# cristicbz/rust-doom

Hardware: NVIDIA H100
Metric: frames/sec at 1920x1080 (palette-index bit-exact) (higher is better)
Workload: dtype u8

## Files before the change

### rust-doom_b200/csrc/b2d_kernels.cu

```cuda
#include "b2d_kernels.cuh"

namespace b2d {

namespace {

constexpr unsigned kFull = 0xFFFFFFFFu;

constexpr int kMaskWords = 128;
constexpr int kStackDepth = 128;

constexpr uint32_t kVisBit = 1u << 25, kSolidBit = 1u << 24;
__device__ __forceinline__ uint32_t pack_range(int lo, int hi, uint32_t bits) {
    return (uint32_t)lo | ((uint32_t)hi << 12) | bits;
}
__device__ __forceinline__ int range_lo(uint32_t r) { return (int)(r & 0xFFFu); }
__device__ __forceinline__ int range_hi(uint32_t r) { return (int)((r >> 12) & 0xFFFu); }

__device__ __forceinline__ uint32_t word_bits(int w, int lo, int hi) {
    int a = max(lo, w * 32), b = min(hi, w * 32 + 31);
    if (a > b) return 0u;
    uint32_t m = 0xFFFFFFFFu >> (31 - (b - w * 32));
    return m & (0xFFFFFFFFu << (a - w * 32));
}

// ... 413 lines not shown
        const uint32_t r = sc.skyrow[y];
        put_px<kRgba>(c, p8, p32, y >= ya && y < yb, __ldg(px + (inter ? (r >> 2) * w4 + (r & 3u) : r * T.w)));
    }
}

template <bool kRgba, int kW>
__device__ __forceinline__ void draw_plane_warp(const RasterCtx &c, const FrameConst &fc, const View &vw,
                                                int ya, int yb, int32_t h, int32_t flat, int lightb,
                                                bool visible) {
    const DeviceScene &sc = *c.sc;
    if (!__any_sync(kFull, ya < yb)) return;
    if (!visible) { fill_void_warp<kRgba, kW>(c, ya, yb); return; }
    if (flat == kFlatSky) { draw_sky_warp<kRgba, kW>(c, ya, yb); return; }
    if (flat < 0 || flat >= sc.nflats) { fill_void_warp<kRgba, kW>(c, ya, yb); return; }
    const uint64_t px_hi = reinterpret_cast<uint64_t>(sc.lit_flats) & 0xFFFFFFFF00000000ull;
    const uint32_t habs = plane_habs(h, fc.pose.z);
    bool act = ya < yb;
    int y0 = __reduce_min_sync(kFull, act ? ya : 0x7FFFFFFF);
    int y1 = __reduce_max_sync(kFull, act ? yb : 0);
    const int full_lo = __reduce_max_sync(kFull, act ? ya : 0x7FFFFFFF);
    const int full_hi = __reduce_min_sync(kFull, act ? yb : 0);
    const int Wc = kW ? kW : c.W;
    uint8_t *p8 = c.fb + (size_t)y0 * Wc;
    uint32_t *p32 = kRgba ? c.rgba + (size_t)y0 * Wc : nullptr;
    const uint32_t bu = (uint32_t)fc.pose.x << 10, bv = (uint32_t)fc.pose.y << 10;
    const uint32_t ax = (uint32_t)c.dir.ax, ay = (uint32_t)c.dir.ay;
    for (int yc = y0; yc < y1; yc += 32) {
        int yy = yc + c.lane;
        if (yy < y1) {
            const PlaneRow pr = plane_row(habs, sc.yslope[yy]);
            c.rowz[c.lane] = make_uint2(pr.z8q, (sc.lit_flat_stride >> 6) * (uint32_t)light_row(lightb, pr.z8) + 64u * (uint32_t)flat);
        }
        __syncwarp();
        const int rows = min(32, y1 - yc);
        int j = 0;
        for (; j + kBatch <= rows; j += kBatch, p8 += (size_t)kBatch * Wc, p32 += (size_t)kBatch * Wc) {
            uint32_t v[kBatch];
#pragma unroll
            for (int k = 0; k < kBatch; k++) {
                const uint2 rz = c.rowz[j + k];
                v[k] = __ldg(reinterpret_cast<const uint8_t *>(px_hi | flat_offset(rz.y, bu + rz.x * ax, bv + rz.x * ay)));
            }
            const int y = yc + j;
            store_batch<kRgba, kW>(c, p8, p32, v, y, ya, yb, y >= full_lo && y + kBatch <= full_hi);
        }
        for (; j < rows; j++, p8 += Wc, p32 += Wc) {
            const uint2 rz = c.rowz[j];
            const int y = yc + j;
            put_px<kRgba>(c, p8, p32, y >= ya && y < yb,
                          __ldg(reinterpret_cast<const uint8_t *>(px_hi | flat_offset(rz.y, bu + rz.x * ax, bv + rz.x * ay))));
        }
        __syncwarp();
    }
}

template <bool kRgba, int kW, int R>
__device__ __forceinline__ void wall_fast_loop(const RasterCtx &c, const uint8_t *plq, uint32_t w4, uint32_t nq, uint32_t q,
                                               uint32_t acc, uint32_t ts29, int y0, int y1, int ya, int yb,
                                               int full_lo, int full_hi) {
    const int Wc = kW ? kW : c.W;
    uint8_t *p8 = c.fb + (size_t)y0 * Wc;
    uint32_t *p32 = kRgba ? c.rgba + (size_t)y0 * Wc : nullptr;
    asm("" : "+l"(plq));
#pragma unroll 1
    for (int y = y0; y < y1; y += R, p8 += (size_t)R * Wc, p32 += (size_t)R * Wc) {
        const uint32_t q1 = q + 1u == nq ? 0u : q + 1u;
        const uint32_t w0 = __ldg(reinterpret_cast<const uint32_t *>(plq + (size_t)q * w4));
        const uint32_t w1 = __ldg(reinterpret_cast<const uint32_t *>(plq + (size_t)q1 * w4));
        if (y >= full_lo && y + R <= full_hi) {
#pragma unroll
            for (int k = 0; k < R; k++) {
                uint32_t v = pick_byte(w0, w1, wall_sel(acc, ts29, (uint32_t)k));
                if (kRgba) v &= 0xFFu;
                put_px<kRgba>(c, p8 + (size_t)k * Wc, kRgba ? p32 + (size_t)k * Wc : nullptr, true, v);
            }
        } else {
            const uint32_t m = row_mask(y, ya, yb, R);
#pragma unroll
            for (int k = 0; k < R; k++) {
                uint32_t v = pick_byte(w0, w1, wall_sel(acc, ts29, (uint32_t)k));
                if (kRgba) v &= 0xFFu;
                put_px<kRgba>(c, p8 + (size_t)k * Wc, kRgba ? p32 + (size_t)k * Wc : nullptr, (m >> k) & 1u, v);
            }
        }
        wall_advance(acc, q, ts29, (uint32_t)R, nq);
    }
}

template <bool kRgba, int kW>
__device__ __forceinline__ void draw_wall_warp(const RasterCtx &c, const FrameConst &fc, int ya, int yb,
                                               int32_t tex, int32_t tA, int32_t hA, int32_t ucol,
                                               int32_t iscale, int row) {
    const DeviceScene &sc = *c.sc;
    if (!__any_sync(kFull, ya < yb)) return;
    if (tex < 0 || tex >= sc.ntex) { fill_void_warp<kRgba, kW>(c, ya, yb); return; }
    const TexRec T = sc.tex[tex];
    bool act = ya < yb;
    const uint32_t col = (uint32_t)floormod32(ucol, (int32_t)T.w);
    const uint8_t *pl = sc.lit_texels + (size_t)row * sc.lit_texel_stride + T.texel_off;
    const uint32_t tstep = (uint32_t)(iscale >> 4);
    int y0 = __reduce_min_sync(kFull, act ? ya : 0x7FFFFFFF);
    int y1 = __reduce_max_sync(kFull, act ? yb : 0);
    const int full_lo = __reduce_max_sync(kFull, act ? ya : 0x7FFFFFFF);
    const int full_hi = __reduce_min_sync(kFull, act ? yb : 0);
    uint32_t t = (uint32_t)wall_tbase(tA, hA, fc.pose.z, c.H, iscale) + (uint32_t)y0 * tstep;
    const int Wc = kW ? kW : c.W;
    uint8_t *p8 = c.fb + (size_t)y0 * Wc;
    uint32_t *p32 = kRgba ? c.rgba + (size_t)y0 * Wc : nullptr;
    if (tex_interleaved(T) && T.h >= 8u) {
        const uint32_t ts = act ? tstep : 0u;
        const bool f16 = __all_sync(kFull, ts <= kWallFast16);
        if (f16 || __all_sync(kFull, ts <= kWallFast8)) {
            const uint32_t tt = act ? t : 0u;
            const uint32_t r0 = wall_row((int32_t)tt, T.h, T.hmagic, T.hbias);
            const uint8_t *plq = pl + 4u * col;
            if (f16) wall_fast_loop<kRgba, kW, 16>(c, plq, 4u * T.w, T.h >> 2, r0 >> 2, wall_acc29(tt, r0), ts << 13, y0, y1, ya, yb, full_lo, full_hi);
            else wall_fast_loop<kRgba, kW, 8>(c, plq, 4u * T.w, T.h >> 2, r0 >> 2, wall_acc29(tt, r0), ts << 13, y0, y1, ya, yb, full_lo, full_hi);
            return;
        }
    }
    if (tex_interleaved(T)) {
        const uint32_t colb = 4u * col, w4 = 4u * T.w;
        for (int y = y0; y < y1; y += kBatch, p8 += (size_t)kBatch * Wc, p32 += (size_t)kBatch * Wc, t += (uint32_t)kBatch * tstep) {
            const uint32_t r0 = wall_row((int32_t)t, T.h, T.hmagic, T.hbias);
            const uint32_t acc = wall_acc(t, r0);
            const uint32_t b7 = (acc + 7u * tstep) >> 16;
            uint32_t v[kBatch];
            if (__all_sync(kFull, b7 < 8u)) {
                const uint32_t q0 = r0 >> 2, q1 = next_quad(q0, T.h);
                const uint32_t w0 = __ldg(reinterpret_cast<const uint32_t *>(pl + (q0 * w4 + colb)));
                const uint32_t w1 = __ldg(reinterpret_cast<const uint32_t *>(pl + (q1 * w4 + colb)));
#pragma unroll
                for (int k = 0; k < kBatch; k++) {
                    v[k] = pick_byte(w0, w1, (acc + (uint32_t)k * tstep) >> 16);
                    if (kRgba) v[k] &= 0xFFu;
                }
            } else {
                const uint32_t t4 = t + 4u * tstep;
                const uint32_t r4 = wall_row((int32_t)t4, T.h, T.hmagic, T.hbias);
                const uint32_t acc4 = wall_acc(t4, r4);
                if (__all_sync(kFull, ((acc + 3u * tstep) >> 16) < 8u && ((acc4 + 3u * tstep) >> 16) < 8u)) {
                    const uint32_t q0 = r0 >> 2, q4 = r4 >> 2;
                    const uint32_t a0 = __ldg(reinterpret_cast<const uint32_t *>(pl + (q0 * w4 + colb)));
                    const uint32_t a1 = __ldg(reinterpret_cast<const uint32_t *>(pl + (next_quad(q0, T.h) * w4 + colb)));
                    const uint32_t b0 = __ldg(reinterpret_cast<const uint32_t *>(pl + (q4 * w4 + colb)));
                    const uint32_t b1 = __ldg(reinterpret_cast<const uint32_t *>(pl + (next_quad(q4, T.h) * w4 + colb)));
#pragma unroll
                    for (int k = 0; k < 4; k++) {
                        v[k] = pick_byte(a0, a1, (acc + (uint32_t)k * tstep) >> 16);
                        v[k + 4] = pick_byte(b0, b1, (acc4 + (uint32_t)k * tstep) >> 16);
                        if (kRgba) { v[k] &= 0xFFu; v[k + 4] &= 0xFFu; }
                    }
                } else {
#pragma unroll
                    for (int k = 0; k < kBatch; k++) {
                        const uint32_t rk = wall_row((int32_t)(t + (uint32_t)k * tstep), T.h, T.hmagic, T.hbias);
                        v[k] = __ldg(pl + ((rk >> 2) * w4 + colb + (rk & 3u)));
                    }
                }
            }
            store_batch<kRgba, kW>(c, p8, p32, v, y, ya, yb, y >= full_lo && y + kBatch <= full_hi);
        }
    } else {
        const uint8_t *px = pl + col;
#pragma unroll 1
        for (int y = y0; y < y1; y++, p8 += Wc, p32 += Wc, t += tstep)
            put_px<kRgba>(c, p8, p32, y >= ya && y < yb, __ldg(px + wall_row((int32_t)t, T.h, T.hmagic, T.hbias) * T.w));
    }
}

__device__ __forceinline__ uint32_t *masked_entry(const DeviceScene &sc, const uint32_t *chunks, int e) {
    return sc.masked_list + ((size_t)chunks[e / kMaskedChunk] * kMaskedChunk + (size_t)(e % kMaskedChunk)) * 33u;
}
__device__ __forceinline__ uint32_t *masked_push(const DeviceScene &sc, uint32_t *chunks, int &mcount, int lane) {
    bool ok = mcount < sc.masked_cap;
    if (ok && mcount % kMaskedChunk == 0) {
        uint32_t id = 0;
        if (lane == 0) id = atomicAdd(sc.masked_counter, 1u);
        id = __shfl_sync(kFull, id, 0);
        ok = id < sc.masked_chunks;
        if (ok && lane == 0) chunks[mcount / kMaskedChunk] = id;
        __syncwarp();
    }
    if (!ok) {
        if (lane == 0) atomicOr(sc.status_flag, kStatusMaskedFull);
        return nullptr;
    }
    return masked_entry(sc, chunks, mcount++);
}

template <bool kRgba, int kW, bool kStates, bool kLevels>
__device__ __noinline__ void masked_pass(const DeviceScene &sc, const View &vw, int32_t pose_z, uint8_t *fb,
                                         uint32_t *rgba, uint32_t pal_s, int x, int lane,
                                         const SegFrame *wl, const uint32_t *chunks, int count) {
    RasterCtx c;
    c.sc = &sc; c.pal_s = pal_s; c.fb = fb; c.rgba = rgba;
    c.W = vw.W; c.H = vw.H; c.x = x; c.lane = lane;
    const int Wc = kW ? kW : c.W;
    for (int e = count - 1; e >= 0; e--) {
        const uint32_t *ml = masked_entry(sc, chunks, e);
        const uint32_t k = ml[0];
        const uint32_t packed = ml[1 + c.lane];
        int ya = (int)(packed & 0xFFFFu), yb = (int)(packed >> 16);
        const SegFrame sf = wl[k];
        int32_t tex, tA, hA, ucol = 0, iscale = 1, row = 0;
        if (is_sprite_entry(sf)) {
            SpriteFrame sp;
            const SpriteRec P = sc.sprites[entry_sprite(sf, sp)];
            if (P.tex < 0 || P.tex >= sc.ntex) continue;
            const int32_t sw = (int32_t)sc.tex[P.tex].w, sh = (int32_t)sc.tex[P.tex].h;
            const int64_t scale = sprite_scale(vw, sp.cz);
            int32_t z8;
            scale_depth(vw, scale, iscale, z8);
            row = light_row_sprite(P.light, z8);
            tex = P.tex; tA = 0; hA = P.low + sh;
            if (ya < yb) {
                clip_rows(P.low + sh, P.low, row_scale(scale), pose_z, c.H, ya, yb);
                ucol = sprite_column(sp, vw, c.x, sw);
            }
        } else {
            const SegRec S = sc.segs[sf.seg];
            if (S.mid < 0 || S.mid >= sc.nmids) continue;
            const MidRec M = sc.mids[S.mid];
            tex = M.tex; tA = M.t_high; hA = M.high;
            ColumnEval ce = {0u, 1, 1, 0};
            if (ya < yb && column_eval(sf, vw, c.x, ce)) {
                clip_rows(M.high, M.low, ce.scale, pose_z, c.H, ya, yb);
                ucol = wall_column(S.uoff, S.len_q12, ce.s24);
                iscale = ce.iscale;
                row = light_row(S.light, ce.z8);
            } else {
                ya = yb = 0;
            }
        }
        if (tex < 0 || tex >= sc.ntex) continue;
        const TexRec T = sc.tex[tex];
        const bool act = ya < yb;
        int y0 = __reduce_min_sync(kFull, act ? ya : 0x7FFFFFFF);
        int y1 = __reduce_max_sync(kFull, act ? yb : 0);
        if (y0 >= y1) continue;
        const uint32_t col = (uint32_t)floormod32(ucol, (int32_t)T.w);
        const bool inter = tex_interleaved(T);
        const bool has_mask = T.mask_off != 0xFFFFFFFFu;
        const uint8_t *pl = sc.lit_texels + (size_t)row * sc.lit_texel_stride + T.texel_off;
        const uint8_t *pm = sc.lit_texels + (size_t)32 * sc.lit_texel_stride + T.texel_off;
        const uint32_t tstep = (uint32_t)(iscale >> 4);
        uint32_t t = (uint32_t)wall_tbase(tA, hA, pose_z, c.H, iscale) + (uint32_t)y0 * tstep;
        uint8_t *p8 = c.fb + (size_t)y0 * Wc;
        uint32_t *p32 = kRgba ? c.rgba + (size_t)y0 * Wc : nullptr;
        const uint32_t len = act ? (uint32_t)(yb - ya) : 0u;
        if (inter) {
            const uint32_t colb = 4u * col, w4 = 4u * T.w;
#pragma unroll 1
            for (int y = y0; y < y1; y += kBatch, p8 += (size_t)kBatch * Wc, p32 += (size_t)kBatch * Wc, t += (uint32_t)kBatch * tstep) {
                const uint32_t r0 = wall_row((int32_t)t, T.h, T.hmagic, T.hbias);
                const uint32_t acc = wall_acc(t, r0);
                const uint32_t d = (uint32_t)(y - ya);
                uint32_t v[kBatch], o[kBatch];
                if (__all_sync(kFull, ((acc + 7u * tstep) >> 16) < 8u)) {
                    const uint32_t o0 = (r0 >> 2) * w4 + colb, o1 = next_quad(r0 >> 2, T.h) * w4 + colb;
                    const uint32_t w0 = __ldg(reinterpret_cast<const uint32_t *>(pl + o0));
                    const uint32_t w1 = __ldg(reinterpret_cast<const uint32_t *>(pl + o1));
                    uint32_t m0 = 0x01010101u, m1 = 0x01010101u;
                    if (has_mask) {
                        m0 = __ldg(reinterpret_cast<const uint32_t *>(pm + o0));
                        m1 = __ldg(reinterpret_cast<const uint32_t *>(pm + o1));
                    }
#pragma unroll
                    for (int k = 0; k < kBatch; k++) {
                        const uint32_t bk = (acc + (uint32_t)k * tstep) >> 16;
                        v[k] = pick_byte(w0, w1, bk) & 0xFFu;
                        o[k] = pick_byte(m0, m1, bk) & 0xFFu;
                    }
                } else {
#pragma unroll
                    for (int k = 0; k < kBatch; k++) {
                        const uint32_t rk = wall_row((int32_t)(t + (uint32_t)k * tstep), T.h, T.hmagic, T.hbias);
                        const uint32_t off = (rk >> 2) * w4 + colb + (rk & 3u);
                        v[k] = __ldg(pl + off);
                        o[k] = has_mask ? (uint32_t)__ldg(pm + off) : 1u;
                    }
                }
#pragma unroll
                for (int k = 0; k < kBatch; k++)
                    put_px<kRgba>(c, p8 + (size_t)k * Wc, kRgba ? p32 + (size_t)k * Wc : nullptr, d + (uint32_t)k < len && o[k] != 0u, v[k]);
            }
        } else {
#pragma unroll 1
            for (int y = y0; y < y1; y++, p8 += Wc, p32 += Wc, t += tstep) {
                const uint32_t off = wall_row((int32_t)t, T.h, T.hmagic, T.hbias) * T.w + col;
                const bool on = (uint32_t)(y - ya) < len && (!has_mask || __ldg(pm + off) != 0);
                put_px<kRgba>(c, p8, p32, on, __ldg(pl + off));
            }
        }
    }
}

constexpr int kRasterWarps = 8;

constexpr uint32_t kQueueWords = 6144;
constexpr uint32_t kQueueRecs = kQueueWords / 32;
constexpr uint32_t kRecWall = 1u << 16, kRecVisible = 1u << 17;

struct DrawQueue {
    uint4 *head;
    uint32_t *pool;
    uint32_t *nrec, *nwords;
};

__device__ __forceinline__ bool queue_push(const DrawQueue &q, int lane, uint32_t meta, int32_t a, int32_t b, int32_t c,
                                           int ya, int yb, int32_t ucol, uint32_t iscale_row) {
    const bool act = ya < yb;
    if (!__any_sync(kFull, act)) return true;
    const bool wall = meta & kRecWall;
    const uint32_t words = wall ? 96u : 32u;
    uint32_t off = 0, i = kQueueRecs;
    if (lane == 0) {
        off = atomicAdd(q.nwords, words);
        if (off + words <= kQueueWords) i = atomicAdd(q.nrec, 1u);
    }
    i = __shfl_sync(kFull, i, 0);
    if (i >= kQueueRecs) return false;
    off = __shfl_sync(kFull, off, 0);
    q.pool[off + lane] = act ? (uint32_t)ya | ((uint32_t)yb << 16) : 0u;
    if (wall) {
        q.pool[off + 32 + lane] = (uint32_t)ucol;
        q.pool[off + 64 + lane] = iscale_row;
    }
    if (lane == 0) q.head[i] = make_uint4(meta | off, (uint32_t)a, (uint32_t)b, (uint32_t)c);
    return true;
}

template <bool kRgba, int kW, bool kMasked, bool kStates, bool kLevels>
__global__ void __launch_bounds__(32 * kRasterWarps, 16 / kRasterWarps)
b2d_raster_kernel(const __grid_constant__ DeviceScene sc, const __grid_constant__ View vw, const FrameConst *__restrict__ frames,
                  const SegFrame *__restrict__ work, int stride, int n, int strips,
                  uint8_t *__restrict__ index_fb, uint32_t *__restrict__ rgba_fb, const __grid_constant__ StateTables st,
                  const __grid_constant__ LevelTables lt) {
    __shared__ uint32_t s_pal[kRgba ? (kLevels ? 256 * kRasterWarps : 256) : 1];
    __shared__ uint2 s_rowz[kRasterWarps][32];
    __shared__ uint32_t s_chunks[kRasterWarps][kMasked ? kMaskedCapMax / kMaskedChunk : 1];
    __shared__ int4 s_lanes[kRasterWarps][32];
    __shared__ int s_frame[kRasterWarps];
    __shared__ uint4 s_qhead[kQueueRecs];
    __shared__ uint32_t s_qpool[kQueueWords];
    __shared__ uint32_t s_qn[3];
    __shared__ DeviceScene s_scn[kStates || kLevels ? kRasterWarps : 1];
    if (threadIdx.x < 3) s_qn[threadIdx.x] = 0;
    if (kRgba && !kLevels) {
        for (int i = threadIdx.x; i < 256; i += blockDim.x) s_pal[i] = sc.palette[i];
    }
    __syncthreads();

    const int lane = threadIdx.x & 31, warp = threadIdx.x >> 5;
    const long long gw = (long long)blockIdx.x * (blockDim.x >> 5) + warp;
    const bool has_strip = gw < (long long)n * strips;
    const int frame = has_strip ? (int)(gw / strips) : 0, strip = has_strip ? (int)(gw % strips) : 0;
    const int W = kW ? kW : vw.W, H = vw.H;
    const int x0 = strip * 32, x = x0 + lane;
    const bool inside = has_strip && x < W;
    const DrawQueue q{s_qhead, s_qpool, &s_qn[0], &s_qn[1]};

    FrameConst fc{};
    if (has_strip) fc = frames[frame];
    const DeviceScene *scp = &sc;
    if constexpr (kStates && !kLevels) {
        DeviceScene *d = &s_scn[warp];
        if (has_strip) {
            const uint32_t *src = reinterpret_cast<const uint32_t *>(&sc);
            uint32_t *dst = reinterpret_cast<uint32_t *>(d);
            for (int i = lane; i < (int)(sizeof(DeviceScene) / 4); i += 32) dst[i] = src[i];
            __syncwarp();
            if (lane == 0) {
                const uint8_t *tb = st.base + (size_t)(uint32_t)fc.pad[0] * st.slot_bytes;
                d->tex = reinterpret_cast<const TexRec *>(tb);
                d->sectors = reinterpret_cast<const SectorRec *>(tb + st.off_sectors);
                d->segs = reinterpret_cast<const SegRec *>(tb + st.off_segs);
                d->sprites = reinterpret_cast<const SpriteRec *>(tb + st.off_sprites);
                d->mids = reinterpret_cast<const MidRec *>(tb + st.off_mids);
            }
            __syncwarp();
        }
        scp = d;
    }
    if constexpr (kLevels) {
        DeviceScene *d = &s_scn[warp];
        if (has_strip) {
            const DeviceScene *lsrc = lt.scenes + (uint32_t)fc.pad[1];
            const uint32_t *src = reinterpret_cast<const uint32_t *>(lsrc);
            uint32_t *dst = reinterpret_cast<uint32_t *>(d);
            for (int i = lane; i < (int)(sizeof(DeviceScene) / 4); i += 32) dst[i] = src[i];
            if (kRgba) {
                const uint32_t *pal = lsrc->palette;
                for (int i = lane; i < 256; i += 32) s_pal[256 * warp + i] = pal[i];
            }
            __syncwarp();
            if constexpr (kStates) {
                if (lane == 0) {
                    const TableSet t = lt.sets[(uint32_t)fc.pad[0]];
                    d->tex = t.tex; d->sectors = t.sectors; d->segs = t.segs; d->sprites = t.sprites; d->mids = t.mids;
                }
                __syncwarp();
            }
        }
        scp = d;
    }
    const DeviceScene &ts = *scp;
    const DeviceScene &ls = kLevels ? ts : sc;
    RasterCtx c;
    c.sc = &ts;
    c.pal_s = (uint32_t)__cvta_generic_to_shared(kLevels ? s_pal + 256 * warp : s_pal);
    c.rowz = s_rowz[warp];
    c.W = W; c.H = H; c.x = x; c.lane = lane;
    int mcount = 0;
    uint32_t *chunks = s_chunks[warp];
    asm("" : "+l"(chunks));
    const SegFrame *wl = work + (size_t)frame * stride;

    if (has_strip) {
    c.dir = plane_dir(fc, vw, inside ? x : 0, ls.invF);
    c.fb = index_fb + (size_t)frame * W * H + (inside ? x : 0);
    c.rgba = kRgba ? rgba_fb + (size_t)frame * W * H + (inside ? x : 0) : nullptr;
    c.skycol = 0;
    if (ls.sky_tex >= 0 && inside) c.skycol = umulhi32(sky_u32(x, vw, fc.pose.angle), ts.tex[ls.sky_tex].w);
    s_lanes[warp][lane] = make_int4(c.dir.ax, c.dir.ay, (int)c.skycol, inside ? x : 0);
    if (lane == 0) s_frame[warp] = frame;

    int ct = 0, cb = inside ? H : 0;
    const bool defer = kMasked && ls.masked_list != nullptr;
    const int count = fc.count;
    const uint32_t owner = (uint32_t)warp << 18;
    bool done = false;

    for (int k0 = 0; k0 < count && !done; k0 += 32) {
        int k = k0 + lane;
        bool overlap = false;
        if (k < count) {
            int xlo = wl[k].xlo, xhi = wl[k].xhi;
            overlap = xhi >= x0 && xlo <= x0 + 31;
        }
        unsigned m = __ballot_sync(kFull, overlap);
        while (m) {
            int j = __ffs(m) - 1;
            m &= m - 1;
            if (!__any_sync(kFull, ct < cb)) { done = true; break; }
            const SegFrame sf = wl[k0 + j];
            bool in = inside && ct < cb && x >= sf.xlo && x <= sf.xhi;
            if (!__any_sync(kFull, in)) continue;
            if (is_sprite_entry(sf)) {
                if (defer) {
                    uint32_t *ml = masked_push(ls, chunks, mcount, lane);
                    if (ml) {
                        if (lane == 0) ml[0] = (uint32_t)(k0 + j);
                        ml[1 + lane] = in ? ((uint32_t)ct | ((uint32_t)cb << 16)) : 0u;
                    }
                }
                continue;
            }
            ColumnEval ce = {0u, 1, 1, 0};
            bool ok = in && column_eval(sf, vw, x, ce);
            if (!__any_sync(kFull, ok)) continue;

            const SegRec S = ts.segs[sf.seg];
            const SectorRec SF = ts.sectors[S.front];
            const int32_t fcl = SF.ceil, ffl = SF.floor;
            const bool two = S.flags & kSegTwoSided;
            const bool ceil_vis = plane_visible(true, fcl, SF.ceil_flat == kFlatSky, fc.pose.z);
            const bool floor_vis = plane_visible(false, ffl, SF.floor_flat == kFlatSky, fc.pose.z);

            WallRows wr = {ct, ct, ct, ct};
            int yend = ct, row = 0;
            int32_t ucol = 0;
            if (ok) {
                row = light_row(S.light, ce.z8);
                ucol = wall_column(S.uoff, S.len_q12, ce.s24);
                wr = wall_rows(fcl, ffl, two, S.otop, S.obot, ce.scale, fc.pose.z, H, ct, cb);
                yend = cb;
            }
#pragma unroll 1
            for (int pz = 0; pz < 2; pz++) {
                const bool top = pz == 0;
                const int ya = ok ? (top ? ct : wr.y4) : 0, yb = ok ? (top ? wr.y1 : yend) : 0;
                const int32_t h = top ? fcl : ffl, flat = top ? SF.ceil_flat : SF.floor_flat;
                const bool vis = top ? ceil_vis : floor_vis;
                if (!queue_push(q, lane, owner | (vis ? kRecVisible : 0u), h, flat, SF.light, ya, yb, 0, 0u))
                    draw_plane_warp<kRgba, kW>(c, fc, vw, ya, yb, h, flat, SF.light, vis);
            }
#pragma unroll 1
            for (int pw = 0; pw < 2; pw++) {
                const bool upper = pw == 0;
                if (!wall_piece(upper, two, fcl, ffl, S.otop, S.obot)) continue;
                const int ya = ok ? (upper ? wr.y1 : wr.y3) : 0, yb = ok ? (upper ? wr.y2 : wr.y4) : 0;
                const int32_t tex = upper ? S.texA : S.texB, tA = upper ? S.tA : S.tB, hA = upper ? S.hA : S.hB;
                if (!queue_push(q, lane, owner | kRecWall, tex, tA, hA, ya, yb, ucol, (uint32_t)ce.iscale | ((uint32_t)row << 24)))
                    draw_wall_warp<kRgba, kW>(c, fc, ya, yb, tex, tA, hA, ucol, ce.iscale, row);
            }
            if (ok) wall_window(two, wr, H, ct, cb);
            if (defer && two && S.mid >= 0) {
                const bool keep = ok && wr.y2 < wr.y3;
                if (__any_sync(kFull, keep)) {
                    uint32_t *ml = masked_push(ls, chunks, mcount, lane);
                    if (ml) {
                        if (lane == 0) ml[0] = (uint32_t)(k0 + j);
                        ml[1 + lane] = keep ? ((uint32_t)wr.y2 | ((uint32_t)wr.y3 << 16)) : 0u;
                    }
                }
            }
        }
    }
    if (!queue_push(q, lane, owner, 0, 0, 0, inside ? ct : 0, inside ? cb : 0, 0, 0u))
        fill_void_warp<kRgba, kW>(c, inside ? ct : 0, inside ? cb : 0);
    }

    __syncthreads();
    const uint32_t nrec = min(s_qn[0], kQueueRecs);
    for (;;) {
        uint32_t i = 0;
        if (lane == 0) i = atomicAdd(&s_qn[2], 1u);
        i = __shfl_sync(kFull, i, 0);
        if (i >= nrec) break;
        const uint4 hd = s_qhead[i];
        const uint32_t off = hd.x & 0xFFFFu, o = hd.x >> 18;
        const int4 ln = s_lanes[o][lane];
        const int f = s_frame[o];
        const FrameConst fo = frames[f];
        RasterCtx d;
        d.sc = kStates || kLevels ? &s_scn[o] : &sc;
        d.pal_s = (uint32_t)__cvta_generic_to_shared(kLevels ? s_pal + 256 * o : s_pal);
        d.rowz = s_rowz[warp];
        d.dir = PlaneDir{ln.x, ln.y};
        d.fb = index_fb + (size_t)f * W * H + ln.w;
        d.rgba = kRgba ? rgba_fb + (size_t)f * W * H + ln.w : nullptr;
        d.W = W; d.H = H; d.x = ln.w; d.lane = lane;
        d.skycol = (uint32_t)ln.z;
        const uint32_t win = s_qpool[off + lane];
        const int ya = (int)(win & 0xFFFFu), yb = (int)(win >> 16);
        if (hd.x & kRecWall) {
            const uint32_t isr = s_qpool[off + 64 + lane];
            draw_wall_warp<kRgba, kW>(d, fo, ya, yb, (int32_t)hd.y, (int32_t)hd.z, (int32_t)hd.w, (int32_t)s_qpool[off + 32 + lane],
                                      (int32_t)(isr & 0xFFFFFFu), (int)(isr >> 24));
        } else {
            draw_plane_warp<kRgba, kW>(d, fo, vw, ya, yb, (int32_t)hd.y, (int32_t)hd.z, (int)hd.w, hd.x & kRecVisible);
        }
    }
    if constexpr (kMasked) {
        __syncthreads();
        if (mcount > 0) masked_pass<kRgba, kW, kStates, kLevels>(ts, vw, fc.pose.z, c.fb, c.rgba, c.pal_s, x, lane, wl, chunks, mcount);
    }
}

__global__ void __launch_bounds__(256)
b2d_palette_kernel(const uint32_t *__restrict__ palette, const uint8_t *__restrict__ index,
                   uint32_t *__restrict__ rgba, size_t n_pixels) {
    __shared__ uint32_t s_pal[256];
    s_pal[threadIdx.x] = palette[threadIdx.x];
    __syncthreads();
    const bool aligned = ((reinterpret_cast<uintptr_t>(index) | reinterpret_cast<uintptr_t>(rgba)) & 15) == 0;
    const size_t nvec = aligned ? n_pixels / 16 : 0;
    const size_t stride = (size_t)gridDim.x * blockDim.x;
    for (size_t i = (size_t)blockIdx.x * blockDim.x + threadIdx.x; i < nvec; i += stride) {
        uint4 in = __ldcs(reinterpret_cast<const uint4 *>(index) + i);
        uint32_t wds[4] = {in.x, in.y, in.z, in.w};
        uint4 *out = reinterpret_cast<uint4 *>(rgba) + 4 * i;
#pragma unroll
        for (int q = 0; q < 4; q++) {
            uint4 o;
            o.x = s_pal[wds[q] & 0xFF];
            o.y = s_pal[(wds[q] >> 8) & 0xFF];
            o.z = s_pal[(wds[q] >> 16) & 0xFF];
            o.w = s_pal[wds[q] >> 24];
            __stcs(out + q, o);
        }
    }
    for (size_t p = nvec * 16 + (size_t)blockIdx.x * blockDim.x + threadIdx.x; p < n_pixels; p += stride)
        rgba[p] = s_pal[index[p]];
}

__global__ void __launch_bounds__(256)
b2d_palette_levels_kernel(const uint32_t *__restrict__ palettes, const uint32_t *__restrict__ tables,
                          const uint8_t *__restrict__ index, uint32_t *__restrict__ rgba, size_t npix, int parts) {
    __shared__ uint32_t s_pal[256];
    const size_t frame = blockIdx.x / parts;
    const int part = blockIdx.x % parts;
    s_pal[threadIdx.x] = palettes[(size_t)tables[frame] * 256 + threadIdx.x];
    __syncthreads();
    const uint8_t *in = index + frame * npix;
    uint32_t *out = rgba + frame * npix;
    const bool aligned = npix % 16 == 0 && ((reinterpret_cast<uintptr_t>(index) | reinterpret_cast<uintptr_t>(rgba)) & 15) == 0;
    const size_t n = aligned ? npix / 16 : npix;
    const size_t per = (n + parts - 1) / parts, lo = (size_t)part * per, hi = lo + per < n ? lo + per : n;
    if (aligned) {
        for (size_t i = lo + threadIdx.x; i < hi; i += blockDim.x) {
            const uint4 q = __ldcs(reinterpret_cast<const uint4 *>(in) + i);
            const uint32_t wds[4] = {q.x, q.y, q.z, q.w};
            uint4 *o4 = reinterpret_cast<uint4 *>(out) + 4 * i;
#pragma unroll
            for (int k = 0; k < 4; k++) {
                uint4 o;
                o.x = s_pal[wds[k] & 0xFF];
                o.y = s_pal[(wds[k] >> 8) & 0xFF];
                o.z = s_pal[(wds[k] >> 16) & 0xFF];
                o.w = s_pal[wds[k] >> 24];
                __stcs(o4 + k, o);
            }
        }
    } else {
        for (size_t p = lo + threadIdx.x; p < hi; p += blockDim.x) out[p] = s_pal[in[p]];
    }
}

constexpr int kResolveRgba = 0, kResolveRgb = 1, kResolvePlanar = 2, kResolveGray = 3;

template <int N>
__device__ __forceinline__ void store_run(uint8_t *dst, const uint32_t (&w)[(N + 3) / 4]) {
    const uintptr_t a = reinterpret_cast<uintptr_t>(dst);
    if constexpr (N % 16 == 0) {
        if ((a & 15) == 0) {
#pragma unroll
            for (int q = 0; q < N / 16; q++) __stcs(reinterpret_cast<uint4 *>(dst) + q, make_uint4(w[4 * q], w[4 * q + 1], w[4 * q + 2], w[4 * q + 3]));
            return;
        }
    }
    if constexpr (N % 8 == 0) {
        if ((a & 7) == 0) {
#pragma unroll
            for (int q = 0; q < N / 8; q++) __stcs(reinterpret_cast<uint2 *>(dst) + q, make_uint2(w[2 * q], w[2 * q + 1]));
            return;
        }
    }
    if constexpr (N % 4 == 0) {
        if ((a & 3) == 0) {
#pragma unroll
            for (int q = 0; q < N / 4; q++) __stcs(reinterpret_cast<unsigned int *>(dst) + q, w[q]);
            return;
        }
    }
    if constexpr (N % 2 == 0) {
        if ((a & 1) == 0) {
#pragma unroll
            for (int q = 0; q < N / 2; q++) reinterpret_cast<uint16_t *>(dst)[q] = (uint16_t)(w[q / 2] >> (16 * (q % 2)));
            return;
        }
    }
#pragma unroll
    for (int b = 0; b < N; b++) dst[b] = (uint8_t)(w[b / 4] >> (8 * (b % 4)));
}

template <int K, int FMT, int P>
__device__ __forceinline__ void resolve_emit(uint8_t *o, size_t opix, int OW, int y, int x0, const uint32_t (&acc0)[P],
                                             const uint32_t (&acc1)[P]) {
    constexpr uint32_t kk = K * K, half = K * K / 2;
    const size_t at = (size_t)y * OW + x0;
    if constexpr (FMT == kResolveGray) {
        uint32_t w[(P + 3) / 4] = {};
#pragma unroll
        for (int p = 0; p < P; p++) w[p / 4] |= ((acc0[p] + half) / kk) << (8 * (p % 4));
        store_run<P>(o + at, w);
    } else {
        uint32_t r[P], g[P], b[P];
#pragma unroll
        for (int p = 0; p < P; p++) {
            r[p] = ((acc0[p] & 0xFFFFu) + half) / kk;
            b[p] = ((acc0[p] >> 16) + half) / kk;
            g[p] = (acc1[p] + half) / kk;
        }
        if constexpr (FMT == kResolveRgba) {
            uint32_t w[P];
#pragma unroll
            for (int p = 0; p < P; p++) w[p] = r[p] | (g[p] << 8) | (b[p] << 16) | 0xFF000000u;
            store_run<4 * P>(o + 4 * at, w);
        } else if constexpr (FMT == kResolveRgb) {
            uint32_t w[(3 * P + 3) / 4] = {};
#pragma unroll
            for (int p = 0; p < P; p++) {
                w[(3 * p) / 4] |= r[p] << (8 * ((3 * p) % 4));
                w[(3 * p + 1) / 4] |= g[p] << (8 * ((3 * p + 1) % 4));
                w[(3 * p + 2) / 4] |= b[p] << (8 * ((3 * p + 2) % 4));
            }
            store_run<3 * P>(o + 3 * at, w);
        } else {
            uint32_t wr[(P + 3) / 4] = {}, wg[(P + 3) / 4] = {}, wb[(P + 3) / 4] = {};
#pragma unroll
            for (int p = 0; p < P; p++) {
                wr[p / 4] |= r[p] << (8 * (p % 4));
                wg[p / 4] |= g[p] << (8 * (p % 4));
                wb[p / 4] |= b[p] << (8 * (p % 4));
            }
            store_run<P>(o + at, wr);
            store_run<P>(o + opix + at, wg);
            store_run<P>(o + 2 * opix + at, wb);
        }
    }
}

template <int K, int FMT>
__global__ void __launch_bounds__(256)
b2d_resolve_kernel(const uint32_t *__restrict__ palettes, const uint32_t *__restrict__ tables, const uint8_t *__restrict__ index,
                   uint8_t *__restrict__ out, int W, int H, int parts, bool vec) {
    constexpr int P = K == 1 ? 16 : K == 2 ? 8 : K == 4 ? 4 : K == 6 ? 8 : K == 8 ? 2 : 16;
    constexpr int kBpp = FMT == kResolveRgba ? 4 : FMT == kResolveGray ? 1 : 3;
    __shared__ uint2 s_tab[256];
    const size_t frame = blockIdx.x / parts;
    const int part = blockIdx.x % parts;
    {
        const uint32_t c = palettes[(size_t)(tables ? tables[frame] : 0u) * 256 + threadIdx.x];
        const uint32_t R = c & 0xFF, G = (c >> 8) & 0xFF, B = (c >> 16) & 0xFF;
        s_tab[threadIdx.x] = FMT == kResolveGray ? make_uint2((77 * R + 150 * G + 29 * B + 128) >> 8, 0u) : make_uint2(R | (B << 16), G);
    }
    __syncthreads();
    const int OW = W / K, OH = H / K;
    const size_t opix = (size_t)OW * OH;
    const uint8_t *in = index + frame * (size_t)W * H;
    uint8_t *o = out + frame * opix * kBpp;
    if (vec) {
        const int groups = OW / P;
        const size_t n = (size_t)OH * groups, per = (n + parts - 1) / parts, lo = (size_t)part * per, hi = lo + per < n ? lo + per : n;
        for (size_t i = lo + threadIdx.x; i < hi; i += blockDim.x) {
            const int y = (int)(i / groups), x0 = (int)(i % groups) * P;
            const uint8_t *src = in + (size_t)y * K * W + (size_t)x0 * K;
            uint32_t acc0[P], acc1[P];
#pragma unroll
            for (int p = 0; p < P; p++) acc0[p] = acc1[p] = 0;
#pragma unroll
            for (int j = 0; j < K; j++) {
#pragma unroll
                for (int q = 0; q < P * K / 16; q++) {
                    const uint4 v = __ldcs(reinterpret_cast<const uint4 *>(src + (size_t)j * W) + q);
                    const uint32_t wds[4] = {v.x, v.y, v.z, v.w};
#pragma unroll
                    for (int b = 0; b < 16; b++) {
                        const uint2 t = s_tab[(wds[b / 4] >> (8 * (b % 4))) & 0xFF];
                        acc0[(16 * q + b) / K] += t.x;
                        if (FMT != kResolveGray) acc1[(16 * q + b) / K] += t.y;
                    }
                }
            }
            resolve_emit<K, FMT, P>(o, opix, OW, y, x0, acc0, acc1);
        }
    } else {
        const size_t n = opix, per = (n + parts - 1) / parts, lo = (size_t)part * per, hi = lo + per < n ? lo + per : n;
        for (size_t i = lo + threadIdx.x; i < hi; i += blockDim.x) {
            const int y = (int)(i / OW), x = (int)(i % OW);
            const uint8_t *src = in + (size_t)y * K * W + (size_t)x * K;
            uint32_t acc0[1] = {0}, acc1[1] = {0};
#pragma unroll
            for (int j = 0; j < K; j++) {
#pragma unroll
                for (int b = 0; b < K; b++) {
                    const uint2 t = s_tab[__ldcs(src + (size_t)j * W + b)];
                    acc0[0] += t.x;
                    if (FMT != kResolveGray) acc1[0] += t.y;
                }
            }
            resolve_emit<K, FMT, 1>(o, opix, OW, y, x, acc0, acc1);
        }
    }
}

}

size_t walk_smem_per_warp(const DeviceScene &sc) { return walk_layout(sc.nverts, sc.nsegs, sc.nnodes, sc.nss, sc.nsprites).total; }

static int device_sms() {
    int dev = 0, sms = 0;
    cudaGetDevice(&dev);
    cudaDeviceGetAttribute(&sms, cudaDevAttrMultiProcessorCount, dev);
    return sms > 0 ? sms : 1;
}

template <bool kStates, bool kLevels>
static cudaError_t walk_go(const BatchTables &t, size_t smem, const View &vw, const Pose *d_poses, int n, FrameConst *d_frames,
                           SegFrame *d_work, int stride, cudaStream_t stream, bool background) {
    if (n <= 0) return cudaSuccess;
    if (smem > 227 * 1024) return cudaErrorInvalidValue;
    if (smem > 48 * 1024) {
        cudaError_t e = cudaFuncSetAttribute(b2d_walk_kernel<kStates, kLevels>, cudaFuncAttributeMaxDynamicSharedMemorySize, (int)smem);
        if (e != cudaSuccess) return e;
    }
    const int sms = device_sms();
    const int blocks = (background && n > sms) ? sms : n, warps = 4;
    b2d_walk_kernel<kStates, kLevels><<<blocks, warps * 32, smem, stream>>>(t.scene, vw, d_poses, n, d_frames, d_work, stride,
                                                                            t.states, t.levels);
    return cudaGetLastError();
}

size_t walk_levels_static_smem() {
    static const size_t bytes = [] {
        cudaFuncAttributes a{}, b{};
        if (cudaFuncGetAttributes(&a, b2d_walk_kernel<false, true>) == cudaSuccess &&
            cudaFuncGetAttributes(&b, b2d_walk_kernel<true, true>) == cudaSuccess)
            return a.sharedSizeBytes > b.sharedSizeBytes ? a.sharedSizeBytes : b.sharedSizeBytes;
        cudaGetLastError();
        return sizeof(DeviceScene) + 16;
    }();
    return bytes;
}

cudaError_t launch_walk(const BatchTables &t, size_t levels_smem, const View &vw, const Pose *d_poses, int n,
                        FrameConst *d_frames, SegFrame *d_work, int stride, cudaStream_t stream, bool background) {
    if (t.per_level && levels_smem + walk_levels_static_smem() > kWalkSmemMax) return cudaErrorInvalidValue;
    const size_t smem = t.per_level ? levels_smem : walk_smem_per_warp(t.scene);
    auto go = t.per_level ? (t.per_frame ? walk_go<true, true> : walk_go<false, true>)
                          : (t.per_frame ? walk_go<true, false> : walk_go<false, false>);
    return go(t, smem, vw, d_poses, n, d_frames, d_work, stride, stream, background);
}

template <bool kStates, bool kLevels>
static cudaError_t raster_go(const BatchTables &t, bool masked, const View &vw, const FrameConst *d_frames,
                             const SegFrame *d_work, int stride, int n, uint8_t *d_index_fb, uint32_t *d_rgba,
                             cudaStream_t stream) {
    if (n <= 0) return cudaSuccess;
    const int strips = (vw.W + 31) / 32;
    const int nblocks = (int)(((long long)n * strips + kRasterWarps - 1) / kRasterWarps);
#define B2D_RASTER_GO(RGBA, KW) do { \
    if (masked) b2d_raster_kernel<RGBA, KW, true, kStates, kLevels><<<nblocks, 32 * kRasterWarps, 0, stream>>>(t.scene, vw, d_frames, d_work, stride, n, strips, d_index_fb, d_rgba, t.states, t.levels); \
    else b2d_raster_kernel<RGBA, KW, false, kStates, kLevels><<<nblocks, 32 * kRasterWarps, 0, stream>>>(t.scene, vw, d_frames, d_work, stride, n, strips, d_index_fb, d_rgba, t.states, t.levels); \
    } while (0)
    if (d_rgba) { if (vw.W == 1920) B2D_RASTER_GO(true, 1920); else B2D_RASTER_GO(true, 0); }
    else if (vw.W == 1920) B2D_RASTER_GO(false, 1920);
    else if (vw.W == 3840) B2D_RASTER_GO(false, 3840);
    else B2D_RASTER_GO(false, 0);
#undef B2D_RASTER_GO
    return cudaGetLastError();
}

cudaError_t launch_raster(const BatchTables &t, bool masked, const View &vw, const FrameConst *d_frames, const SegFrame *d_work,
                          int stride, int n, uint8_t *d_index_fb, uint32_t *d_rgba, cudaStream_t stream) {
    auto go = t.per_level ? (t.per_frame ? raster_go<true, true> : raster_go<false, true>)
                          : (t.per_frame ? raster_go<true, false> : raster_go<false, false>);
    return go(t, masked, vw, d_frames, d_work, stride, n, d_index_fb, d_rgba, stream);
}

namespace {
__global__ void __launch_bounds__(256)
b2d_prelight_kernel(const uint8_t *__restrict__ colormap, const uint8_t *__restrict__ src, uint8_t *__restrict__ dst,
                    size_t n, size_t stride) {
    __shared__ uint8_t cm[32 * 256];
    for (int i = threadIdx.x; i < 32 * 256; i += blockDim.x) cm[i] = colormap[i];
    __syncthreads();
// ... 144 lines not shown
```

Measured before the change: 550,000.

## Split raster queue records into vertical row bands for finer warp load balancing

Each queued wall/plane record now stores its min/max row span, and after the queue is built the block counts, prefix-sums and scatters (record, 256-row band) items into shared memory. Warps then pull band items instead of whole records and clip their row window to the band, so a tall record can be drawn by several warps in parallel. This targets tail imbalance where one warp draws a long column while the others idle. It adds two extra block syncs, shared-memory atomics and per-item setup overhead, and falls back to whole records when items overflow or masked work exists.

```diff
diff --git a/rust-doom_b200/csrc/b2d_kernels.cu b/rust-doom_b200/csrc/b2d_kernels.cu
--- a/rust-doom_b200/csrc/b2d_kernels.cu
+++ b/rust-doom_b200/csrc/b2d_kernels.cu
@@ -739,8 +739,14 @@
 constexpr uint32_t kQueueRecs = kQueueWords / 32;
 constexpr uint32_t kRecWall = 1u << 16, kRecVisible = 1u << 17;
 
+constexpr int kBandRows = 256;
+constexpr int kMaxBands = (2160 + kBandRows - 1) / kBandRows;
+constexpr uint32_t kItemCap = 1024;
+static_assert(kBandRows % 32 == 0 && kMaxBands <= 256 && kQueueRecs <= 256, "an item is record | band << 8 in 16 bits");
+
 struct DrawQueue {
     uint4 *head;
+    uint32_t *ext;
     uint32_t *pool;
     uint32_t *nrec, *nwords;
 };
@@ -749,6 +755,8 @@
                                            int ya, int yb, int32_t ucol, uint32_t iscale_row) {
     const bool act = ya < yb;
     if (!__any_sync(kFull, act)) return true;
+    const uint32_t y0 = __reduce_min_sync(kFull, act ? (uint32_t)ya : 0xFFFFu);
+    const uint32_t y1 = __reduce_max_sync(kFull, act ? (uint32_t)yb : 0u);
     const bool wall = meta & kRecWall;
     const uint32_t words = wall ? 96u : 32u;
     uint32_t off = 0, i = kQueueRecs;
@@ -764,7 +772,10 @@
         q.pool[off + 32 + lane] = (uint32_t)ucol;
         q.pool[off + 64 + lane] = iscale_row;
     }
-    if (lane == 0) q.head[i] = make_uint4(meta | off, (uint32_t)a, (uint32_t)b, (uint32_t)c);
+    if (lane == 0) {
+        q.head[i] = make_uint4(meta | off, (uint32_t)a, (uint32_t)b, (uint32_t)c);
+        q.ext[i] = y0 | y1 << 16;
+    }
     return true;
 }
 
@@ -780,10 +791,14 @@
     __shared__ int4 s_lanes[kRasterWarps][32];
     __shared__ int s_frame[kRasterWarps];
     __shared__ uint4 s_qhead[kQueueRecs];
+    __shared__ uint32_t s_qext[kQueueRecs];
     __shared__ uint32_t s_qpool[kQueueWords];
-    __shared__ uint32_t s_qn[3];
+    __shared__ uint16_t s_items[kItemCap];
+    __shared__ uint32_t s_band[kMaxBands];
+    __shared__ uint32_t s_qn[5];
     __shared__ DeviceScene s_scn[kStates || kLevels ? kRasterWarps : 1];
-    if (threadIdx.x < 3) s_qn[threadIdx.x] = 0;
+    if (threadIdx.x < 5) s_qn[threadIdx.x] = 0;
+    for (int b = threadIdx.x; b < kMaxBands; b += blockDim.x) s_band[b] = 0;
     if (kRgba && !kLevels) {
         for (int i = threadIdx.x; i < 256; i += blockDim.x) s_pal[i] = sc.palette[i];
     }
@@ -796,7 +811,7 @@
     const int W = kW ? kW : vw.W, H = vw.H;
     const int x0 = strip * 32, x = x0 + lane;
     const bool inside = has_strip && x < W;
-    const DrawQueue q{s_qhead, s_qpool, &s_qn[0], &s_qn[1]};
+    const DrawQueue q{s_qhead, s_qext, s_qpool, &s_qn[0], &s_qn[1]};
 
     FrameConst fc{};
     if (has_strip) fc = frames[frame];
@@ -949,13 +964,61 @@
         fill_void_warp<kRgba, kW>(c, inside ? ct : 0, inside ? cb : 0);
     }
 
+    if (kMasked && mcount > 0 && lane == 0) s_qn[4] = 1;
     __syncthreads();
     const uint32_t nrec = min(s_qn[0], kQueueRecs);
+    for (uint32_t r = threadIdx.x; r < nrec; r += blockDim.x) {
+        const uint32_t e = s_qext[r];
+        for (uint32_t b = (e & 0xFFFFu) / kBandRows; b <= ((e >> 16) - 1u) / kBandRows; b++) atomicAdd(&s_band[b], 1u);
+    }
+    __syncthreads();
+    if (warp == 0) {
+        constexpr int kPer = (kMaxBands + 31) / 32;
+        uint32_t v[kPer], sum = 0;
+#pragma unroll
+        for (int k = 0; k < kPer; k++) {
+            const int b = lane * kPer + k;
+            v[k] = b < kMaxBands ? s_band[b] : 0u;
+            sum += v[k];
+        }
+        uint32_t incl = sum;
+#pragma unroll
+        for (int d = 1; d < 32; d <<= 1) {
+            const uint32_t u = __shfl_up_sync(kFull, incl, d);
+            if (lane >= d) incl += u;
+        }
+        uint32_t at = incl - sum;
+#pragma unroll
+        for (int k = 0; k < kPer; k++) {
+            const int b = lane * kPer + k;
+            if (b < kMaxBands) s_band[b] = at;
+            at += v[k];
+        }
+        if (lane == 31) s_qn[3] = incl;
+    }
+    __syncthreads();
+    const bool banded = s_qn[3] <= kItemCap && !(kMasked && s_qn[4]);
+    if (banded) {
+        for (uint32_t r = threadIdx.x; r < nrec; r += blockDim.x) {
+            const uint32_t e = s_qext[r];
+            for (uint32_t b = (e & 0xFFFFu) / kBandRows; b <= ((e >> 16) - 1u) / kBandRows; b++)
+                s_items[atomicAdd(&s_band[b], 1u)] = (uint16_t)(r | b << 8);
+        }
+        __syncthreads();
+    }
+    const uint32_t nitems = banded ? s_qn[3] : nrec;
     for (;;) {
         uint32_t i = 0;
         if (lane == 0) i = atomicAdd(&s_qn[2], 1u);
         i = __shfl_sync(kFull, i, 0);
-        if (i >= nrec) break;
+        if (i >= nitems) break;
+        int lo = 0, hi = H;
+        if (banded) {
+            const uint32_t it = s_items[i];
+            i = it & 0xFFu;
+            lo = (int)(it >> 8) * kBandRows;
+            hi = lo + kBandRows;
+        }
         const uint4 hd = s_qhead[i];
         const uint32_t off = hd.x & 0xFFFFu, o = hd.x >> 18;
         const int4 ln = s_lanes[o][lane];
@@ -971,7 +1034,7 @@
         d.W = W; d.H = H; d.x = ln.w; d.lane = lane;
         d.skycol = (uint32_t)ln.z;
         const uint32_t win = s_qpool[off + lane];
-        const int ya = (int)(win & 0xFFFFu), yb = (int)(win >> 16);
+        const int ya = max((int)(win & 0xFFFFu), lo), yb = min((int)(win >> 16), hi);
         if (hd.x & kRecWall) {
             const uint32_t isr = s_qpool[off + 64 + lane];
             draw_wall_warp<kRgba, kW>(d, fo, ya, yb, (int32_t)hd.y, (int32_t)hd.z, (int32_t)hd.w, (int32_t)s_qpool[off + 32 + lane],
```

Result: faster. 617,600, median of 6 (+12.3%).
